# HongwenZhang/DaNet-DensePose2SMPL

Hardware: NVIDIA H100
Metric: images/sec DaNet fwd bs=64 224x224 (HRNet-W48 + part regressors + SMPL LBS + IUV render) (higher is better)
Workload: dtype split-f16 operands (hi+lo, 22 bits; 3 MMAs per K step), f32 accumulate

## Files before the change

### __graft_entry__.py

```python
import os
import subprocess
import sys

ROOT = os.path.dirname(os.path.abspath(__file__))
PKG = os.path.join(ROOT, "danet-densepose2smpl_b200")
CSRC = os.path.join(PKG, "csrc")
LIB = os.path.join(PKG, "libdanet_b200.so")
SOURCES = ["api.cu", "lbs.cu", "raster.cu", "glue.cu", "conv_simt.cu", "conv_tc.cu", "net.cu", "losses.cu", "iuv_train.cu",
           "gcn_train.cu", "conv_wgrad.cu", "bn_train.cu"]
ARCH = ["-gencode", "arch=compute_90a,code=sm_90a"]
NVCC_FLAGS = ARCH + [ "-lineinfo", "-O3", "-std=c++17",
              "-Xcompiler", "-fPIC", "--use_fast_math=false"]


def _stale(target, deps):
    if not os.path.exists(target):
        return True
    t = os.path.getmtime(target)
    return any(os.path.getmtime(d) > t for d in deps)


def build(verbose=False):
    nvcc = os.environ.get("NVCC", "/usr/local/cuda/bin/nvcc")
    hdrs = [os.path.join(CSRC, "common.cuh"), os.path.join(ROOT, "include", "danet_b200.h")]
# ... 9 lines not shown
            subprocess.check_call(cmd)
        objs.append(o)
    if _stale(LIB, objs):
        subprocess.check_call([nvcc, "-shared"] + ARCH + ["-o", LIB] + objs + ["-lcudart"])
    exe = os.path.join(ROOT, "examples", "net_host")
    if _stale(exe, [exe + ".c", LIB, os.path.join(ROOT, "include", "danet_b200.h")]):
        subprocess.check_call(["gcc", "-O2", "-I" + os.path.join(ROOT, "include"), exe + ".c", "-o", exe, "-L" + PKG, "-ldanet_b200",
                               "-Wl,-rpath,$ORIGIN/../" + os.path.basename(PKG)])
    subprocess.check_call(["make", "-s", "-C", os.path.join(ROOT, "oracle"), "liboracle.so"])
    if os.path.isdir("/root/reference/models/danet") and not os.path.exists(os.path.join(ROOT, "oracle", "_ref", ".complete")):
        subprocess.check_call([sys.executable, "-m", "oracle.make_ref"], cwd=ROOT)
    if ROOT not in sys.path:
        sys.path.insert(0, ROOT)
    import danet_b200
    return LIB


def smoke():
    if ROOT not in sys.path:
        sys.path.insert(0, ROOT)
    import numpy as np
    import torch
    import danet_b200
    from oracle import synth, lbs as olbs, raster as oraster

    assert torch.cuda.is_available(), "smoke() needs a GPU"
    dev = torch.device("cuda:0")
    model = synth.make_smpl_model(0)
    mesh = synth.make_dp_mesh(0)
    smpl = danet_b200.SMPL(model, batch_size=4).to(dev)
# ... 24 lines not shown
    assert plan.n_tc > 300 and plan.precision == "exact", "smoke must run the tensor-core path"
    kps_err = float((out["stn_kps_pred"].cpu() - torch.from_numpy(g["stn_kps"])).abs().max())
    idx = out["visualization"]["iuv_pred"][2].argmax(1).cpu().numpy()
    parts = out["visualization"]["part_iuv_pred"][:, :, 2].argmax(2).cpu().numpy()
    clean = ~((idx != g["index_argmax"]).reshape(2, -1).any(1) | (parts != g["part_argmax"]).reshape(2, -1).any(1))
    perr = np.abs(out["para"].cpu().numpy() - g["para"]).max(1)
    assert kps_err < 1e-4, kps_err
    assert clean.any() and perr[clean].max() < 1e-4, (perr, clean)
    torch.cuda.synchronize()
    print("smoke ok: verts max|d|=%.2e joints max|d|=%.2e, IUV parts bit-exact, network para max|d|=%.2e (wgmma exact mode, "
          "%d convolutions) vs the reference golden" % (dv, dj, perr[clean].max(), plan.n_tc))


if __name__ == "__main__":
    build(verbose="-v" in sys.argv)
    if "smoke" in sys.argv:
        smoke()
```

### danet-densepose2smpl_b200/csrc/conv_tc.cu

```cuda
#include "common.cuh"
#include "wgmma_f16.cuh"
#include "tc_ptx.cuh"
#include <cuda.h>
#include <cuda_fp16.h>
#include <mutex>
#include <type_traits>
#include <utility>
#include <string.h>
#include <math.h>

namespace danet {
namespace tc {

constexpr int kTileH = 16, kTileW = 8;
__host__ __device__ constexpr int kConsumersOf(int ex) { return ex ? 4 : 2; }
__host__ __device__ constexpr int kThreadsOf(int ex) { return ex ? 4 * 4 * 32 : (4 * 2 + 1) * 32; }
constexpr int kWarpProd = 4 * kConsumersOf(0);
constexpr int kNtMaxExact = 64, kNtMaxFast = 256;
constexpr int kMaxAStages = 8, kMaxBStages = 8;
constexpr int kSmemMax = 227 * 1024;
constexpr int kSmemFixed = 2048;
constexpr int kSchedDepth = 4, kSchedAhead = 2, kSchedStatic = 3;
__host__ __device__ constexpr int kSchedConsumersOf(int ex) { return 4 * kConsumersOf(ex); }
constexpr int kPackHeader = 1024;
constexpr int kSegMmas = 8;

struct alignas(64) Prob {
    CUtensorMap tm[2];
    const uint8_t* wpk; const float* bias;
    const float* res_f; const __half* res_hi; const __half* res_lo;
    float* y_f; __half* y_hi; __half* y_lo;
    int N, H, W, Cin, Cout, Ho, Wo, ks, stride, pad, relu, wsets, exact;
    int npa;
    int SWB, KCH, nchunks;
    int TG;
    int NT, ntn;
    int nstack, hs, box_h;
    int bpc;
    int par_py[4], par_px[4], ntap[4], ngrp[4], stage_bytes[4], sbo_a[4];
    int tapoff16[4][16];
    int tapidx[4][16];
    int tiles_w, tiles_h, tile_count, tile_base;
    int rows_blk;
    int tap_bytes, b_block_bytes, nblk;
    long long blocks_per_set;
    unsigned long long m_ntn, m_tw, m_th, m_ws;
};

constexpr int kMaxProb = 6;
struct ArgsN {
    int nprob, total_tiles, na_stages, a_slot_bytes, nb_stages, b_slot_bytes;
    unsigned* sched;
    Prob p[kMaxProb];
    int pair_base[kMaxProb], pair_count[kMaxProb], total_pairs;
};

static unsigned long long magic40(int d) { return (1ull << 40) / (unsigned long long)d + 1ull; }

static bool make_prob(const danet_conv_desc* d, Prob* g) {
    if (!(d->stride == 1 || d->stride == 2) || !(d->ksize == 1 || d->ksize == 3 || d->ksize == 7) || d->pad != d->ksize / 2) return false;
    if (d->Cin % 8 != 0 || d->Cout % 8 != 0 || d->H < 1 || d->W < 1 || d->N < 1 || d->wsets < 1) return false;
    g->N = d->N; g->H = d->H; g->W = d->W; g->Cin = d->Cin; g->Cout = d->Cout; g->ks = d->ksize;
    g->pad = d->pad; g->stride = d->stride; g->relu = d->relu; g->wsets = d->wsets;
    g->exact = (d->flags & DANET_CONV_EXACT) ? 1 : 0;
    g->Ho = (d->H + 2 * d->pad - d->ksize) / d->stride + 1;
    g->Wo = (d->W + 2 * d->pad - d->ksize) / d->stride + 1;
    if (g->Ho < 1 || g->Wo < 1) return false;
    const int np = (d->Cout + 15) / 16 * 16;
    const int ntmax = g->exact ? kNtMaxExact : kNtMaxFast;
// ... 71 lines not shown
}

static bool plan_rings(ArgsN* a) {
    int amax = 0, bmax = 0, need_a = 2, max_a = kMaxAStages;
    bool exact = false;
    for (int i = 0; i < a->nprob; ++i) {
        const int sb = max_stage_bytes(a->p[i]);
        amax = sb > amax ? sb : amax;
        bmax = a->p[i].b_block_bytes > bmax ? a->p[i].b_block_bytes : bmax;
        if (a->p[i].exact) exact = true;
    }
    a->a_slot_bytes = (amax + 1023) / 1024 * 1024;
    a->b_slot_bytes = (bmax + 1023) / 1024 * 1024;
    if (exact) {
        a->a_slot_bytes *= 2;
        need_a = max_a = 3;
    }
    int nb = 3;
    int na = (kSmemMax - kSmemFixed - nb * a->b_slot_bytes) / a->a_slot_bytes;
    if (na < need_a) { nb = 2; na = (kSmemMax - kSmemFixed - nb * a->b_slot_bytes) / a->a_slot_bytes; }
    if (na < need_a) return false;
    if (na > max_a) na = max_a;
    while (nb < kMaxBStages && kSmemFixed + na * a->a_slot_bytes + (nb + 1) * a->b_slot_bytes <= kSmemMax) ++nb;
    a->na_stages = na; a->nb_stages = nb;
    return true;
}

__device__ __forceinline__ uint64_t make_desc(uint32_t saddr, uint32_t sbo_bytes, uint32_t swb) {
    const uint32_t mode = swb == 128 ? 1u : (swb == 64 ? 2u : 3u);
    const uint32_t lo = ((saddr >> 4) & 0x3FFFu) | (1u << 16);
    const uint32_t hi = ((sbo_bytes >> 4) & 0x3FFFu) | (mode << 30);
// ... 31 lines not shown
    if (g.tiles_h > 1) {
        const int th2 = (g.tiles_h + 1) >> 1;
        grp = outer / th2;
        c.th = 2 * (outer - grp * th2) + h;
    } else {
        const int q = mdiv(outer, g.m_ws);
        grp = (2 * q + h) * g.wsets + (outer - q * g.wsets);
        c.th = 0;
    }
    const int bg = mdiv(grp, g.m_ws);
    c.ws = grp - bg * g.wsets;
    c.img0 = c.ws + g.wsets * bg * g.nstack;
    return c;
}

struct Ring { int as, bs; uint32_t aph, bph; };

struct Smem { uint32_t sA, sB, bar_a_full, bar_a_empty, bar_b_full, bar_b_empty; };

constexpr uint32_t kOffSchedFull = 512, kOffSchedEmpty = kOffSchedFull + 8 * kSchedDepth;
constexpr uint32_t kOffSchedRing = kOffSchedFull + 16 * kSchedDepth, kOffCursor = 640, kOffPark = 768;

enum CursorField {
    kCurSeq, kCurPub, kCurPubEnd,
    kCurPi,
    kCurC, kCurSlot, kCurStep,
    kCurH0, kCurH1, kCurW0,
    kCurImg0, kCurImg1, kCurBlk,
    kCurFa, kCurFb,
    kCurRa, kCurRb,
    kCurAs, kCurBs, kCurAph, kCurBph,
    kCurFields
};
static_assert(kOffCursor + 4 * kCurFields <= kOffPark && kOffPark + 4 * 32 <= 1024, "barrier region layout");
__device__ __forceinline__ int cur_get(uint32_t cur, int f) {
    int v;
    asm volatile("ld.shared.s32 %0, [%1];" : "=r"(v) : "r"(cur + 4 * f) : "memory");
    return v;
}
__device__ __forceinline__ void cur_set(uint32_t cur, int f, int v) {
    asm volatile("st.shared.s32 [%0], %1;" ::"r"(cur + 4 * f), "r"(v) : "memory");
}

__device__ __forceinline__ void produce(const ArgsN& a, const Smem& S, int dA, int dB) {
    const uint32_t cur = S.bar_a_full + kOffCursor;
    cur_set(cur, kCurRa, cur_get(cur, kCurRa) + dA);
    cur_set(cur, kCurRb, cur_get(cur, kCurRb) + dB);
#pragma unroll 1
    for (;;) {
        if (cur_get(cur, kCurPi) < 0) {
#pragma unroll 1
            while (cur_get(cur, kCurPub) <= cur_get(cur, kCurSeq) + kSchedAhead && !cur_get(cur, kCurPubEnd)) {
                const int pub = cur_get(cur, kCurPub), rs = pub & (kSchedDepth - 1);
                mbar_wait_inl(S.bar_a_full + kOffSchedEmpty + 8 * rs, ((pub / kSchedDepth) & 1) ^ 1);
                int t;
                if (pub < kSchedStatic || !a.sched) t = (int)blockIdx.x + pub * (int)gridDim.x;
                else t = __shfl_sync(0xffffffffu, atom_inc_elect(a.sched), 0) + kSchedStatic * (int)gridDim.x;
                if (t >= a.total_pairs) { t = a.total_pairs; cur_set(cur, kCurPubEnd, 1); }
                st_arrive_elect(S.bar_a_full + kOffSchedRing + 4 * rs, t, S.bar_a_full + kOffSchedFull + 8 * rs);
                cur_set(cur, kCurPub, pub + 1);
            }
            int pair;
            asm volatile("ld.shared.s32 %0, [%1];" : "=r"(pair)
                         : "r"(S.bar_a_full + kOffSchedRing + 4 * (cur_get(cur, kCurSeq) & (kSchedDepth - 1))) : "memory");
            pair = __shfl_sync(0xffffffffu, pair, 0);
            if (pair >= a.total_pairs) return;
            int pi = 0;
            while (pair >= a.pair_base[pi] + a.pair_count[pi]) ++pi;
            const Prob& P = a.p[pi];
            const int pp = pair - a.pair_base[pi];
            {
                const TileCoord tc = pair_coord(P, pp, 0);
                cur_set(cur, kCurH0, tc.th * kTileH * P.stride - P.pad);
                cur_set(cur, kCurW0, tc.tw * kTileW * P.stride - P.pad);
                cur_set(cur, kCurImg0, tc.img0);
                cur_set(cur, kCurBlk, tc.ws * (int)P.blocks_per_set + tc.nt * P.nblk);
            }
            {
                const TileCoord tc = pair_coord(P, pp, 1);
                cur_set(cur, kCurH1, tc.th * kTileH * P.stride - P.pad);
                cur_set(cur, kCurImg1, tc.img0);
            }
            cur_set(cur, kCurC, 0); cur_set(cur, kCurSlot, 0); cur_set(cur, kCurStep, 0);
            cur_set(cur, kCurPi, pi);
        }
        const Prob& P = a.p[cur_get(cur, kCurPi)];
        const int step = cur_get(cur, kCurStep);
        if (step < 2) {
            if (cur_get(cur, kCurFa) >= cur_get(cur, kCurRa) + a.na_stages) return;
            {
                const int as = cur_get(cur, kCurAs);
                mbar_wait_inl(S.bar_a_empty + 8 * as, ((cur_get(cur, kCurAph) >> as) & 1) ^ 1);
                mbar_expect_tx_elect(S.bar_a_full + 8 * as, 2u * P.nstack * P.box_h * P.sbo_a[cur_get(cur, kCurSlot)]);
            }
#pragma unroll 1
            for (int k = 0; k < 2 * P.nstack; ++k) {
                const int h = k >= P.nstack ? 1 : 0, n = k - h * P.nstack, slot = cur_get(cur, kCurSlot), as = cur_get(cur, kCurAs);
                tma_load_4d_elect(S.sA + as * a.a_slot_bytes + h * (a.a_slot_bytes >> 1) + n * P.hs * P.sbo_a[slot],
                                  &P.tm[step], cur_get(cur, kCurC) * P.KCH, cur_get(cur, kCurW0) + P.par_px[slot],
                                  cur_get(cur, kCurH0 + h) + P.par_py[slot], cur_get(cur, kCurImg0 + h) + n * P.wsets,
                                  S.bar_a_full + 8 * as);
            }
            const int as = cur_get(cur, kCurAs);
            cur_set(cur, kCurAph, cur_get(cur, kCurAph) ^ (1 << as));
            cur_set(cur, kCurAs, as + 1 == a.na_stages ? 0 : as + 1);
            cur_set(cur, kCurFa, cur_get(cur, kCurFa) + 1);
            cur_set(cur, kCurStep, step + 1);
        } else {
            if (cur_get(cur, kCurFb) >= cur_get(cur, kCurRb) + a.nb_stages) return;
            {
                const int bs = cur_get(cur, kCurBs);
                mbar_wait_inl(S.bar_b_empty + 8 * bs, ((cur_get(cur, kCurBph) >> bs) & 1) ^ 1);
                const uint32_t bar = S.bar_b_full + 8 * bs;
                mbar_expect_tx_elect(bar, (uint32_t)P.b_block_bytes);
                bulk_g2s_elect(S.sB + bs * a.b_slot_bytes, P.wpk + kPackHeader + (long long)cur_get(cur, kCurBlk) * P.b_block_bytes,
                               (uint32_t)P.b_block_bytes, bar);
                cur_set(cur, kCurBph, cur_get(cur, kCurBph) ^ (1 << bs));
                cur_set(cur, kCurBs, bs + 1 == a.nb_stages ? 0 : bs + 1);
            }
            cur_set(cur, kCurFb, cur_get(cur, kCurFb) + 1);
            cur_set(cur, kCurBlk, cur_get(cur, kCurBlk) + 1);
            const int slot = cur_get(cur, kCurSlot);
            if (step - 1 < P.ngrp[slot]) cur_set(cur, kCurStep, step + 1);
            else {
                cur_set(cur, kCurStep, 0);
                if (slot + 1 < P.npa) cur_set(cur, kCurSlot, slot + 1);
                else {
                    cur_set(cur, kCurSlot, 0);
                    if (cur_get(cur, kCurC) + 1 < P.nchunks) cur_set(cur, kCurC, cur_get(cur, kCurC) + 1);
                    else { cur_set(cur, kCurPi, -1); cur_set(cur, kCurSeq, cur_get(cur, kCurSeq) + 1); }
                }
            }
        }
    }
}

template <int EX, int NT>
__device__ __forceinline__ void consume_tile(const ArgsN& a, const Prob& P, const TileCoord tc, const Smem S, Ring& R,
                                             int wg, int w4, int lane, bool leader, float* accs, float* sum,
                                             int half = 0, bool prod = false) {
    constexpr int NV = NT / 2;
    constexpr int nj = NT / 8;
    const int prow0 = 8 * wg + 2 * w4, pcol = lane >> 2, cq = 2 * (lane & 3);
    float* s = accs;
    float* m = EX ? accs + NV : accs;
    const int Cout = P.Cout, Wo = P.Wo, Ho = P.Ho;
    const int cw = Cout - tc.nt * NT;
    uint32_t eoff[2]; bool ok[2];
    const int ow = tc.tw * kTileW + pcol;
#pragma unroll
    for (int r = 0; r < 2; ++r) {
        const int prow = prow0 + r;
        int oh = tc.th * kTileH + prow, img = tc.img0;
        bool row_ok = oh < Ho;
        if (P.nstack > 1) {
// ... 26 lines not shown
                    }
                }
            }
        }
        return t;
    };
    if constexpr (EX) {
#pragma unroll
        for (int j = 0; j < nj; ++j)
#pragma unroll
            for (int r = 0; r < 2; ++r) {
                const float2 t = init_term(j, r);
                sum[4 * j + 2 * r] = t.x * wsc.x; sum[4 * j + 2 * r + 1] = t.y * wsc.x;
            }
    }
    using Var = std::conditional_t<EX, int, const int>;
    Var nchunks = P.nchunks, npa = P.npa, TG = P.TG, SWB = P.SWB;
    Var kmma = P.KCH / 16;
    std::conditional_t<EX, int, const uint32_t> tap16 = P.tap_bytes >> 4;
    std::conditional_t<EX, int, const uint32_t> hi16 = EX ? (NT * SWB) >> 4 : 0;
    const uint64_t bd0 = make_desc(0, 8 * SWB, SWB);
    uint32_t acc = 0;
    int seg_cnt = 0;
    int pend_b = -1, pend_a = -1;
    auto release_pending = [&]() {
        mbar_arrive_if(S.bar_b_empty + 8 * pend_b, leader && pend_b >= 0);
        mbar_arrive_if(S.bar_a_empty + 8 * pend_a, leader && pend_a >= 0);
        pend_b = pend_a = -1;
    };
    for (int c = 0; c < nchunks; ++c) {
        const int kreal = (P.Cin - c * P.KCH + 15) >> 4;
        Var kv = kreal < kmma ? kreal : kmma;
        for (int slot = 0; slot < npa; ++slot) {
            Var as_hi = R.as;
            mbar_wait_inl(S.bar_a_full + 8 * R.as, (R.aph >> R.as) & 1u);
            R.aph ^= 1u << R.as; if (++R.as == a.na_stages) R.as = 0;
            int as_lo = as_hi;
            if (EX) {
                as_lo = R.as;
                mbar_wait_inl(S.bar_a_full + 8 * R.as, (R.aph >> R.as) & 1u);
                R.aph ^= 1u << R.as; if (++R.as == a.na_stages) R.as = 0;
            }
            const uint64_t ad0 = make_desc(0, (uint32_t)P.sbo_a[slot], SWB) + ((uint32_t)(wg * 8 * P.sbo_a[slot]) >> 4);
            const uint64_t ad_hi = ad0 + ((S.sA + as_hi * a.a_slot_bytes) >> 4);
            Var ngrp = P.ngrp[slot], ntap = P.ntap[slot];
            for (int tg = 0; tg < ngrp; ++tg) {
                const int k0 = tg * TG;
                const int ntk = min(TG, ntap - k0);
                const int bs = R.bs;
                mbar_wait_inl(S.bar_b_full + 8 * bs, (R.bph >> bs) & 1u);
                R.bph ^= 1u << bs; if (++R.bs == a.nb_stages) R.bs = 0;
                uint64_t bd;
                if constexpr (EX) bd = make_desc(0, 8 * SWB, SWB) + ((S.sB + bs * a.b_slot_bytes) >> 4);
                else bd = bd0 + ((S.sB + bs * a.b_slot_bytes) >> 4);
                wg_fence();
                if constexpr (EX) {
                    const uint32_t tile_a = S.sA + half * (a.a_slot_bytes >> 1) + wg * 8 * P.sbo_a[slot];
                    const uint64_t ad1 = make_desc(0, (uint32_t)P.sbo_a[slot], SWB);
                    const uint64_t ad_hi = ad1 + ((tile_a + as_hi * a.a_slot_bytes) >> 4);
                    const uint64_t ad_lo = ad1 + ((tile_a + as_lo * a.a_slot_bytes) >> 4);
                    #pragma unroll 1
                    for (int tt = 0; tt < ntk; ++tt) {
                        const uint32_t toff = (uint32_t)P.tapoff16[slot][k0 + tt];
                        #pragma unroll
                        for (int kk = 0; kk < 4; ++kk) {
// ... 12 lines not shown
                        }
                    }
                } else {
                    #pragma unroll 1
                    for (int tt = 0; tt < ntk; ++tt) {
                        const uint32_t toff = (uint32_t)P.tapoff16[slot][k0 + tt];
                        #pragma unroll
                        for (int kk = 0; kk < 4; ++kk) {
                            if (kk >= kv) break;
                            Wgmma<NT>::mma(m, m + NT / 4, ad_hi + toff + 2 * kk, bd + tt * tap16 + 2 * kk, acc);
                            acc = 1;
                        }
                    }
                }
                wg_commit();
                const bool plane_end = tg == ngrp - 1;
                if constexpr (EX) {
                    seg_cnt += ntk * kv;
                    const bool close = (c == nchunks - 1 && slot == npa - 1 && plane_end) || seg_cnt >= kSegMmas;
                    const int db = pend_b >= 0 ? 1 : 0;
                    int dA = 0, dB = db;
                    if (close || plane_end) {
                        wg_wait_all();
                        reg_fence<NV>(m);
                        reg_fence<NV>(s);
                        if (close) {
#pragma unroll
                            for (int j = 0; j < NV; ++j) {
                                sum[j] += m[j];
                                sum[j] += s[j];
                            }
                            acc = 0; seg_cnt = 0;
                        }
                        release_pending();
                        mbar_arrive_if(S.bar_b_empty + 8 * bs, leader);
                        mbar_arrive_if(S.bar_a_empty + 8 * as_hi, leader && plane_end);
                        mbar_arrive_if(S.bar_a_empty + 8 * as_lo, leader && plane_end);
                        dA = plane_end ? 2 : 0; dB = db + 1;
                    } else {
                        wg_wait_1();
                        release_pending();
                        pend_b = bs;
                    }
                    if (prod) {
                        const uint32_t pk = S.bar_a_full + kOffPark;
                        int* const v[] = {&c, &slot, &tg, &kv, &ngrp, &ntap, &as_hi, &as_lo, &seg_cnt, &pend_b, &R.as, &R.bs,
                                          &nchunks, &npa, &TG, &SWB, &kmma, &tap16, &hi16};
                        constexpr int nv = sizeof(v) / sizeof(v[0]);
#pragma unroll
                        for (int i = 0; i < nv; ++i) cur_set(pk, i, *v[i]);
                        cur_set(pk, nv, (int)acc); cur_set(pk, nv + 1, (int)R.aph); cur_set(pk, nv + 2, (int)R.bph);
                        produce(a, S, dA, dB);
#pragma unroll
                        for (int i = 0; i < nv; ++i) *v[i] = __shfl_sync(0xffffffffu, cur_get(pk, i), 0);
                        acc = (uint32_t)__shfl_sync(0xffffffffu, cur_get(pk, nv), 0);
                        R.aph = (uint32_t)__shfl_sync(0xffffffffu, cur_get(pk, nv + 1), 0);
                        R.bph = (uint32_t)__shfl_sync(0xffffffffu, cur_get(pk, nv + 2), 0);
                    }
                } else {
                    wg_wait_1();
                    release_pending();
                    pend_b = bs;
                    if (plane_end) pend_a = as_hi;
                }
            }
        }
    }
    wg_wait_all();
    reg_fence<NV>(m);
    if constexpr (EX) reg_fence<NV>(s);
    release_pending();
    const int relu = P.relu;
    float* __restrict__ y_f = P.y_f; __half* __restrict__ y_hi = P.y_hi; __half* __restrict__ y_lo = P.y_lo;
#pragma unroll
    for (int j = 0; j < nj; ++j) {
        if (8 * j >= cw) continue;
#pragma unroll
        for (int r = 0; r < 2; ++r) {
            if (!ok[r]) continue;
            float v0, v1;
            if constexpr (EX) { v0 = sum[4 * j + 2 * r]; v1 = sum[4 * j + 2 * r + 1]; }
            else {
                const float2 t = init_term(j, r);
                v0 = m[4 * j + 2 * r]; v1 = m[4 * j + 2 * r + 1];
                v0 += t.x * wsc.x; v1 += t.y * wsc.x;
            }
            float x0 = v0 * wsc.y, x1 = v1 * wsc.y;
            if (relu) { x0 = fmaxf(x0, 0.f); x1 = fmaxf(x1, 0.f); }
            const uint32_t e = eoff[r] + 8 * j;
            if (y_f) *reinterpret_cast<float2*>(y_f + e) = make_float2(x0, x1);
            if (y_hi) {
                const uint32_t hv = pack_h2_rn(x0, x1);
                *reinterpret_cast<uint32_t*>(y_hi + e) = hv;
                if (y_lo) {
                    const float2 t = h2_to_f2(hv);
                    *reinterpret_cast<uint32_t*>(y_lo + e) = pack_h2_rn(x0 - t.x, x1 - t.y);
                }
            }
        }
    }
}

template <int EX>
__global__ void __launch_bounds__(kThreadsOf(EX), 1)
k_conv_tc(const __grid_constant__ ArgsN a) {
    extern __shared__ __align__(1024) uint8_t smem[];
    const uint32_t sbase = (smem_u32(smem) + 1023u) & ~1023u;
    const uint32_t sA = sbase;
    const uint32_t sB = sbase + a.na_stages * a.a_slot_bytes;
    const uint32_t sBar = sB + a.nb_stages * a.b_slot_bytes;
    const uint32_t bar_a_full = sBar, bar_a_empty = sBar + 8 * kMaxAStages;
    const uint32_t bar_b_full = sBar + 16 * kMaxAStages, bar_b_empty = bar_b_full + 8 * kMaxBStages;
    const uint32_t bar_sched_full = sBar + kOffSchedFull, bar_sched_empty = sBar + kOffSchedEmpty, sched_ring = sBar + kOffSchedRing;
    constexpr int kCons = kConsumersOf(EX);

    const int warp = __shfl_sync(0xffffffffu, (int)(threadIdx.x >> 5), 0), lane = threadIdx.x & 31;
    if (threadIdx.x == 0) {
        for (int i = 0; i < a.na_stages; ++i) { mbar_init(bar_a_full + 8 * i, 1); mbar_init(bar_a_empty + 8 * i, kCons); }
        for (int i = 0; i < a.nb_stages; ++i) { mbar_init(bar_b_full + 8 * i, 1); mbar_init(bar_b_empty + 8 * i, kCons); }
        for (int i = 0; i < kSchedDepth; ++i) { mbar_init(bar_sched_full + 8 * i, 1); mbar_init(bar_sched_empty + 8 * i, kSchedConsumersOf(EX)); }
        asm volatile("fence.mbarrier_init.release.cluster;" ::: "memory");
        if constexpr (EX)
            for (int f = 0; f < kCurFields; ++f) cur_set(sBar + kOffCursor, f, f == kCurPi ? -1 : 0);
    }
    if (warp == (EX ? 0 : kWarpProd) && lane < a.nprob) { tma_prefetch_desc(&a.p[lane].tm[0]); if (EX) tma_prefetch_desc(&a.p[lane].tm[1]); }
    __syncthreads();
    pdl_launch_dependents();

    if constexpr (EX) {
        const int wg = warp >> 2, w4 = warp & 3;
        const bool leader = (threadIdx.x & 127) == 0;
        const bool prod = warp == 0;
        const Smem S = {sA, sB, bar_a_full, bar_a_empty, bar_b_full, bar_b_empty};
        Ring R = {0, 0, 0u, 0u};
        constexpr int NVMAX = kNtMaxExact / 2;
        float accs[2 * NVMAX];
        float sum[NVMAX];
        pdl_wait();
        if (prod) produce(a, S, 0, 0);
        for (int seq = 0;; ++seq) {
            int pair = 0;
            if (lane == 0) pair = sched_next(bar_sched_full, bar_sched_empty, sched_ring, seq);
            pair = __shfl_sync(0xffffffffu, pair, 0);
            if (pair >= a.total_pairs) break;
            int pi = 0;
            while (pair >= a.pair_base[pi] + a.pair_count[pi]) ++pi;
            const Prob& P = a.p[pi];
            const int half = wg >> 1;
            const TileCoord tc = pair_coord(P, pair - a.pair_base[pi], half);
#define DANET_NT_CASE(N) case N: consume_tile<EX, N>(a, P, tc, S, R, wg & 1, w4, lane, leader, accs, sum, half, prod); break;
            switch (P.NT) {
                DANET_NT_CASE(16) DANET_NT_CASE(32) DANET_NT_CASE(48) DANET_NT_CASE(64)
                default: __trap();
            }
#undef DANET_NT_CASE
        }
    } else if (warp == kWarpProd) {
        if (lane == 0) {
            int as = 0, bs = 0; uint32_t aph = 0, bph = 0;
            int pub = 0; bool ended = false;
            for (int seq = 0;; ++seq) {
                while (pub <= seq + kSchedAhead && !ended) {
                    const int slot = pub & (kSchedDepth - 1);
                    mbar_wait(bar_sched_empty + 8 * slot, ((pub / kSchedDepth) & 1) ^ 1);
                    int t;
                    if (pub < kSchedStatic || !a.sched) t = (int)blockIdx.x + pub * (int)gridDim.x;
                    else t = (int)atomicAdd(a.sched, 1u) + kSchedStatic * (int)gridDim.x;
                    if (t >= a.total_tiles) { t = a.total_tiles; ended = true; }
                    asm volatile("st.shared.s32 [%0], %1;" ::"r"(sched_ring + 4 * slot), "r"(t) : "memory");
                    mbar_arrive(bar_sched_full + 8 * slot);
// ... 35 lines not shown
                        }
                    }
            }
        }
    } else {
        const int wg = warp >> 2, w4 = warp & 3;
        const bool leader = (threadIdx.x & 127) == 0;
        const Smem S = {sA, sB, bar_a_full, bar_a_empty, bar_b_full, bar_b_empty};
        Ring R = {0, 0, 0u, 0u};
        float accs[kNtMaxFast / 2];
        pdl_wait();
        for (int seq = 0;; ++seq) {
            int tile = 0;
            if (lane == 0) tile = sched_next(bar_sched_full, bar_sched_empty, sched_ring, seq);
            tile = __shfl_sync(0xffffffffu, tile, 0);
            if (tile >= a.total_tiles) break;
            int pi = 0;
            while (tile >= a.p[pi].tile_base + a.p[pi].tile_count) ++pi;
            const Prob& P = a.p[pi];
            const TileCoord tc = decode_tile(P, tile - P.tile_base);
#define DANET_NT_CASE(N) case N: consume_tile<EX, N>(a, P, tc, S, R, wg, w4, lane, leader, accs, nullptr); break;
            switch (P.NT) {
                DANET_NT_CASE(16) DANET_NT_CASE(32) DANET_NT_CASE(48) DANET_NT_CASE(64) DANET_NT_CASE(80) DANET_NT_CASE(96)
                DANET_NT_CASE(112) DANET_NT_CASE(128) DANET_NT_CASE(144) DANET_NT_CASE(160) DANET_NT_CASE(176) DANET_NT_CASE(192)
                DANET_NT_CASE(208) DANET_NT_CASE(224) DANET_NT_CASE(240) DANET_NT_CASE(256)
                default: __trap();
            }
#undef DANET_NT_CASE
        }
    }
    __syncthreads();
    if (threadIdx.x == 0 && a.sched) {
        __threadfence();
        if (atomicAdd(a.sched + 1, 1u) == gridDim.x - 1) { a.sched[0] = 0u; a.sched[1] = 0u; __threadfence(); }
    }
}

__global__ void k_absmax(long long n, const float* __restrict__ w, unsigned* __restrict__ out) {
    unsigned m = 0;
    for (long long i = (long long)blockIdx.x * blockDim.x + threadIdx.x; i < n; i += (long long)gridDim.x * blockDim.x) {
        const unsigned b = __float_as_uint(fabsf(w[i]));
        if (b < 0x7f800000u && b > m) m = b;
    }
    for (int o = 16; o > 0; o >>= 1) m = max(m, __shfl_xor_sync(0xffffffffu, m, o));
    if ((threadIdx.x & 31) == 0 && m) atomicMax(out, m);
}
// ... 75 lines not shown
    const CUtensorMapSwizzle sw = g.SWB == 128 ? CU_TENSOR_MAP_SWIZZLE_128B : (g.SWB == 64 ? CU_TENSOR_MAP_SWIZZLE_64B : CU_TENSOR_MAP_SWIZZLE_32B);
    const CUresult r = fn(tm, CU_TENSOR_MAP_DATA_TYPE_FLOAT16, 4, const_cast<void*>(base), gdim, gstr, box, estr,
                          CU_TENSOR_MAP_INTERLEAVE_NONE, sw, CU_TENSOR_MAP_L2_PROMOTION_L2_128B, CU_TENSOR_MAP_FLOAT_OOB_FILL_NONE);
    DANET_CHECK(r == CUDA_SUCCESS, "conv_tc: cuTensorMapEncodeTiled failed (%d) for [%d,%d,%d,%d] box [%u,%u,%u]", (int)r,
                g.N, g.H, g.W, g.Cin, box[0], box[1], box[2]);
    return 0;
}

}

static int g_sm_count[64];
static unsigned* g_sched[64];
static unsigned g_sched_seq[64];
constexpr int kSchedSlots = 1024;
static std::mutex g_tc_mu;
static unsigned long long g_tc_devs = 0;

static int configure_group(int n, const danet_conv_desc* const* descs, tc::ArgsN* a) {
    using namespace tc;
    memset(a, 0, sizeof(*a));
    a->nprob = n;
    for (int i = 0; i < n; ++i)
        if (!make_prob(descs[i], &a->p[i])) { set_error("danet_conv_tc_group: problem %d has an unsupported shape", i); return -1; }
    for (int i = 1; i < n; ++i)
        DANET_CHECK(a->p[i].exact == a->p[0].exact, "danet_conv_tc_group: exact and fast problems cannot share a launch");
    DANET_CHECK(plan_rings(a), "danet_conv_tc_group: shared-memory plan does not fit");
    return 0;
}

int conv_tc_group_launch(int n, const danet_conv_problem* probs, cudaStream_t stream) {
// ... 40 lines not shown
    const int units = a.p[0].exact ? a.total_pairs : a.total_tiles;
    int dev = 0;
    DANET_CUDA(cudaGetDevice(&dev));
    DANET_CHECK(dev >= 0 && dev < 64, "conv_tc: device ordinal %d out of range", dev);
    {
        std::lock_guard<std::mutex> lk(g_tc_mu);
        if (first_use_on_current_device(&g_tc_devs) != 0) {
            DANET_CUDA(cudaDeviceGetAttribute(&g_sm_count[dev], cudaDevAttrMultiProcessorCount, dev));
            DANET_CUDA(cudaFuncSetAttribute(k_conv_tc<0>, cudaFuncAttributeMaxDynamicSharedMemorySize, kSmemMax));
            DANET_CUDA(cudaFuncSetAttribute(k_conv_tc<1>, cudaFuncAttributeMaxDynamicSharedMemorySize, kSmemMax));
            DANET_CUDA(cudaMalloc((void**)&g_sched[dev], kSchedSlots * 2 * sizeof(unsigned)));
            DANET_CUDA(cudaMemset(g_sched[dev], 0, kSchedSlots * 2 * sizeof(unsigned)));
        }
        a.sched = g_sched[dev] + 2 * (g_sched_seq[dev]++ % kSchedSlots);
    }
    const int smem_bytes = kSmemFixed + a.na_stages * a.a_slot_bytes + a.nb_stages * a.b_slot_bytes;
    const int cap = g_sm_count[dev];
    const int grid = units < cap ? units : cap;
    cudaLaunchConfig_t cfg = {};
    cfg.gridDim = dim3(grid); cfg.blockDim = dim3(kThreadsOf(a.p[0].exact));
    cfg.dynamicSmemBytes = smem_bytes;
    cfg.stream = stream;
    cudaLaunchAttribute at[1];
    at[0].id = cudaLaunchAttributeProgrammaticStreamSerialization;
    at[0].val.programmaticStreamSerializationAllowed = 1;
    cfg.attrs = at; cfg.numAttrs = 1;
    if (a.p[0].exact) { DANET_CUDA(cudaLaunchKernelEx(&cfg, k_conv_tc<1>, a)); }
    else { DANET_CUDA(cudaLaunchKernelEx(&cfg, k_conv_tc<0>, a)); }
    DANET_LAUNCH_CHECK();
    return 0;
// ... 90 lines not shown
extern "C" int danet_act_split(int64_t n, const float* x, void* hi, void* lo, danet_stream_t stream) {
    DANET_CHECK(n >= 0 && (n == 0 || (x && hi)), "danet_act_split: bad arguments");
    if (n == 0) return 0;
    tc::k_act_split<<<(unsigned)((n + 255) / 256), 256, 0, (cudaStream_t)stream>>>(n, x, (__half*)hi, (__half*)lo);
    DANET_LAUNCH_CHECK();
    return 0;
}

extern "C" int danet_act_merge(int64_t n, const void* hi, const void* lo, float* y, danet_stream_t stream) {
    DANET_CHECK(n >= 0 && (n == 0 || (hi && y)), "danet_act_merge: bad arguments");
    if (n == 0) return 0;
    tc::k_act_merge<<<(unsigned)((n + 255) / 256), 256, 0, (cudaStream_t)stream>>>(n, (const __half*)hi, (const __half*)lo, y);
    DANET_LAUNCH_CHECK();
    return 0;
}
```

Measured before the change: 1562.

## Pack producer cursor state, prefetch next schedule slot, add phase profiler build

Adds an optional phase-profiling build, off by default, that times each consumer phase with clock counters in shared memory. In the default path it also changes the exact-mode producer/consumer loop. Cursor fields are regrouped so they can be read and written with 128-bit shared loads and stores. The parked consumer state shrinks from about 22 words to two bit-packed words, with per-problem constants reloaded from the parameter struct. The next scheduler entry is now fetched before the epilogue rather than after it. The aim is to cut shared-memory traffic and scheduler latency in the interleaved producer role, at the risk of bit-field overflow if stage counts or chunk indices exceed the packed widths.

Result: faster. 1608 (median of 6 runs) (+2.9%).

```diff
diff --git a/__graft_entry__.py b/__graft_entry__.py
--- a/__graft_entry__.py
+++ b/__graft_entry__.py
@@ -47,6 +47,24 @@
         sys.path.insert(0, ROOT)
     import danet_b200
     return LIB
+
+
+PHASE_LIB = os.path.join(PKG, "libdanet_b200_phase.so")
+
+
+def build_phase_profile():
+    build()
+    nvcc = os.environ.get("NVCC", "/usr/local/cuda/bin/nvcc")
+    flags = [f for f in NVCC_FLAGS if not f.startswith("--use_fast_math")]
+    src = os.path.join(CSRC, "conv_tc.cu")
+    obj = os.path.join(PKG, "build", "conv_tc_phase.o")
+    hdrs = [os.path.join(ROOT, "include", "danet_b200.h")] + [os.path.join(CSRC, f) for f in os.listdir(CSRC) if f.endswith(".cuh")]
+    if _stale(obj, [src] + hdrs):
+        subprocess.check_call([nvcc] + flags + ["-DDANET_CONV_PHASE_PROFILE", "-c", src, "-o", obj])
+    objs = [obj if s == "conv_tc.cu" else os.path.join(PKG, "build", s.replace(".cu", ".o")) for s in SOURCES]
+    if _stale(PHASE_LIB, objs):
+        subprocess.check_call([nvcc, "-shared"] + ARCH + ["-o", PHASE_LIB] + objs + ["-lcudart"])
+    return PHASE_LIB
 
 
 def smoke():
@@ -101,5 +119,7 @@
 
 if __name__ == "__main__":
     build(verbose="-v" in sys.argv)
+    if "phase" in sys.argv:
+        build_phase_profile()
     if "smoke" in sys.argv:
         smoke()
diff --git a/danet-densepose2smpl_b200/csrc/conv_tc.cu b/danet-densepose2smpl_b200/csrc/conv_tc.cu
--- a/danet-densepose2smpl_b200/csrc/conv_tc.cu
+++ b/danet-densepose2smpl_b200/csrc/conv_tc.cu
@@ -19,10 +19,15 @@
 constexpr int kNtMaxExact = 64, kNtMaxFast = 256;
 constexpr int kMaxAStages = 8, kMaxBStages = 8;
 constexpr int kSmemMax = 227 * 1024;
+#ifdef DANET_CONV_PHASE_PROFILE
+constexpr int kSmemFixed = 4096;
+#else
 constexpr int kSmemFixed = 2048;
+#endif
 constexpr int kSchedDepth = 4, kSchedAhead = 2, kSchedStatic = 3;
 __host__ __device__ constexpr int kSchedConsumersOf(int ex) { return 4 * kConsumersOf(ex); }
 constexpr int kPackHeader = 1024;
+constexpr int kExactAStages = 3;
 constexpr int kSegMmas = 8;
 
 struct alignas(64) Prob {
@@ -53,6 +58,9 @@
     unsigned* sched;
     Prob p[kMaxProb];
     int pair_base[kMaxProb], pair_count[kMaxProb], total_pairs;
+#ifdef DANET_CONV_PHASE_PROFILE
+    unsigned long long* prof;
+#endif
 };
 
 static unsigned long long magic40(int d) { return (1ull << 40) / (unsigned long long)d + 1ull; }
@@ -154,7 +162,7 @@
     a->b_slot_bytes = (bmax + 1023) / 1024 * 1024;
     if (exact) {
         a->a_slot_bytes *= 2;
-        need_a = max_a = 3;
+        need_a = max_a = kExactAStages;
     }
     int nb = 3;
     int na = (kSmemMax - kSmemFixed - nb * a->b_slot_bytes) / a->a_slot_bytes;
@@ -216,6 +224,50 @@
     return c;
 }
 
+#define DANET_CONV_PHASES(X) \
+    X(Last) X(Start) X(Resident) X(Other) X(Sched) X(Prologue) X(WaitAHi) X(WaitALo) X(WaitB) X(Mma) X(Wait1) X(DrainSeg) X(DrainPlane) X(Sum) \
+    X(Park) X(Produce) X(ProduceSpin) X(Reload) X(Epilogue) X(Tail) X(Units) X(Blocks)
+enum Phase {
+#define X(n) kPh##n,
+    DANET_CONV_PHASES(X)
+#undef X
+    kPhN
+};
+#ifdef DANET_CONV_PHASE_PROFILE
+static_assert(kPhLast == 0 && kPhStart == 1 && kPhResident == 2 && kPhN <= 32, "one lane per phase");
+constexpr uint32_t kOffProf = 1024;
+static_assert(kOffProf + 16 * 4 * kPhN + 1023 <= kSmemFixed, "phase rows");
+__device__ __forceinline__ uint32_t prof_row(uint32_t sbar) { return sbar + kOffProf + (threadIdx.x >> 5) * (4 * kPhN); }
+__device__ __forceinline__ void prof_tick(uint32_t sbar, int ph) {
+    asm volatile("{\n\t.reg .u32 now, prev, sum;\n\tmov.u32 now, %%clock;\n\tld.shared.u32 prev, [%0];\n\tld.shared.u32 sum, [%1];\n\t"
+                 "sub.u32 prev, now, prev;\n\tadd.u32 sum, sum, prev;\n\tst.shared.u32 [%1], sum;\n\tst.shared.u32 [%0], now;\n\t}"
+                 ::"r"(prof_row(sbar)), "r"(prof_row(sbar) + 4 * ph) : "memory");
+}
+__device__ __forceinline__ void prof_count(uint32_t sbar, int ph) {
+    asm volatile("{\n\t.reg .u32 n;\n\tld.shared.u32 n, [%0];\n\tadd.u32 n, n, 1;\n\tst.shared.u32 [%0], n;\n\t}"
+                 ::"r"(prof_row(sbar) + 4 * ph) : "memory");
+}
+__device__ __forceinline__ void prof_start(uint32_t sbar) {
+    asm volatile("{\n\t.reg .pred p;\n\t.reg .u32 now;\n\tsetp.lt.u32 p, %1, %2;\n\t@p st.shared.u32 [%0], 0;\n\tbar.warp.sync 0xffffffff;\n\t"
+                 "mov.u32 now, %%clock;\n\tst.shared.u32 [%3], now;\n\tst.shared.u32 [%3 + 4], now;\n\t}"
+                 ::"r"(prof_row(sbar) + 4 * (threadIdx.x & 31)), "r"(threadIdx.x & 31), "r"((uint32_t)kPhN), "r"(prof_row(sbar)) : "memory");
+}
+__device__ __forceinline__ void prof_flush(uint32_t sbar, unsigned long long* tab, int pi) {
+    const uint32_t lane = threadIdx.x & 31;
+    unsigned long long* dst = tab + ((size_t)pi * 16 + (threadIdx.x >> 5)) * kPhN + lane;
+    const uint32_t on = lane > kPhStart && lane < kPhN && tab != nullptr;
+    asm volatile("{\n\t.reg .pred p;\n\t.reg .u32 v;\n\t.reg .u64 w;\n\tbar.warp.sync 0xffffffff;\n\tsetp.ne.u32 p, %1, 0;\n\t"
+                 "mov.u32 v, 0;\n\t@p ld.shared.u32 v, [%0];\n\tcvt.u64.u32 w, v;\n\t@p red.global.add.u64 [%2], w;\n\t"
+                 "@p st.shared.u32 [%0], 0;\n\tbar.warp.sync 0xffffffff;\n\t}"
+                 ::"r"(prof_row(sbar) + 4 * lane), "r"(on), "l"(dst) : "memory");
+}
+#define PROF_TICK(sbar, ph) prof_tick(sbar, ph)
+#define PROF_COUNT(sbar, ph) prof_count(sbar, ph)
+#else
+#define PROF_TICK(sbar, ph) ((void)0)
+#define PROF_COUNT(sbar, ph) ((void)0)
+#endif
+
 struct Ring { int as, bs; uint32_t aph, bph; };
 
 struct Smem { uint32_t sA, sB, bar_a_full, bar_a_empty, bar_b_full, bar_b_empty; };
@@ -224,17 +276,17 @@
 constexpr uint32_t kOffSchedRing = kOffSchedFull + 16 * kSchedDepth, kOffCursor = 640, kOffPark = 768;
 
 enum CursorField {
+    kCurPi, kCurStep, kCurSlot, kCurC,
+    kCurFb, kCurRb, kCurBs, kCurBph,
+    kCurFa, kCurRa, kCurAs, kCurAph,
+    kCurBlk, kCurW0, kCurH0, kCurH1,
+    kCurImg0, kCurImg1,
     kCurSeq, kCurPub, kCurPubEnd,
-    kCurPi,
-    kCurC, kCurSlot, kCurStep,
-    kCurH0, kCurH1, kCurW0,
-    kCurImg0, kCurImg1, kCurBlk,
-    kCurFa, kCurFb,
-    kCurRa, kCurRb,
-    kCurAs, kCurBs, kCurAph, kCurBph,
     kCurFields
 };
-static_assert(kOffCursor + 4 * kCurFields <= kOffPark && kOffPark + 4 * 32 <= 1024, "barrier region layout");
+static_assert(kOffCursor % 16 == 0 && kCurStep == kCurPi + 1 && kCurSlot == kCurPi + 2 && kCurC == kCurPi + 3 && kCurPi % 4 == 0 &&
+              kCurFb % 4 == 0 && kCurFa % 4 == 0, "cursor groups");
+static_assert(kOffCursor + 4 * kCurFields <= kOffPark && kOffPark + 4 * 2 <= 1024, "barrier region layout");
 __device__ __forceinline__ int cur_get(uint32_t cur, int f) {
     int v;
     asm volatile("ld.shared.s32 %0, [%1];" : "=r"(v) : "r"(cur + 4 * f) : "memory");
@@ -243,18 +295,29 @@
 __device__ __forceinline__ void cur_set(uint32_t cur, int f, int v) {
     asm volatile("st.shared.s32 [%0], %1;" ::"r"(cur + 4 * f), "r"(v) : "memory");
 }
+__device__ __forceinline__ int4 cur_get4(uint32_t cur, int f) {
+    int4 v;
+    asm volatile("ld.shared.v4.s32 {%0, %1, %2, %3}, [%4];" : "=r"(v.x), "=r"(v.y), "=r"(v.z), "=r"(v.w) : "r"(cur + 4 * f) : "memory");
+    return v;
+}
+__device__ __forceinline__ void cur_set4(uint32_t cur, int f, int4 v) {
+    asm volatile("st.shared.v4.s32 [%0], {%1, %2, %3, %4};" ::"r"(cur + 4 * f), "r"(v.x), "r"(v.y), "r"(v.z), "r"(v.w) : "memory");
+}
 
 __device__ __forceinline__ void produce(const ArgsN& a, const Smem& S, int dA, int dB) {
     const uint32_t cur = S.bar_a_full + kOffCursor;
-    cur_set(cur, kCurRa, cur_get(cur, kCurRa) + dA);
-    cur_set(cur, kCurRb, cur_get(cur, kCurRb) + dB);
+    if (dA) cur_set(cur, kCurRa, cur_get(cur, kCurRa) + dA);
+    if (dB) cur_set(cur, kCurRb, cur_get(cur, kCurRb) + dB);
 #pragma unroll 1
     for (;;) {
-        if (cur_get(cur, kCurPi) < 0) {
+        int4 ctl = cur_get4(cur, kCurPi);
+        if (ctl.x < 0) {
 #pragma unroll 1
             while (cur_get(cur, kCurPub) <= cur_get(cur, kCurSeq) + kSchedAhead && !cur_get(cur, kCurPubEnd)) {
                 const int pub = cur_get(cur, kCurPub), rs = pub & (kSchedDepth - 1);
+                PROF_TICK(S.bar_a_full, kPhProduce);
                 mbar_wait_inl(S.bar_a_full + kOffSchedEmpty + 8 * rs, ((pub / kSchedDepth) & 1) ^ 1);
+                PROF_TICK(S.bar_a_full, kPhProduceSpin);
                 int t;
                 if (pub < kSchedStatic || !a.sched) t = (int)blockIdx.x + pub * (int)gridDim.x;
                 else t = __shfl_sync(0xffffffffu, atom_inc_elect(a.sched), 0) + kSchedStatic * (int)gridDim.x;
@@ -283,56 +346,57 @@
                 cur_set(cur, kCurH1, tc.th * kTileH * P.stride - P.pad);
                 cur_set(cur, kCurImg1, tc.img0);
             }
-            cur_set(cur, kCurC, 0); cur_set(cur, kCurSlot, 0); cur_set(cur, kCurStep, 0);
-            cur_set(cur, kCurPi, pi);
-        }
-        const Prob& P = a.p[cur_get(cur, kCurPi)];
-        const int step = cur_get(cur, kCurStep);
-        if (step < 2) {
-            if (cur_get(cur, kCurFa) >= cur_get(cur, kCurRa) + a.na_stages) return;
-            {
-                const int as = cur_get(cur, kCurAs);
-                mbar_wait_inl(S.bar_a_empty + 8 * as, ((cur_get(cur, kCurAph) >> as) & 1) ^ 1);
-                mbar_expect_tx_elect(S.bar_a_full + 8 * as, 2u * P.nstack * P.box_h * P.sbo_a[cur_get(cur, kCurSlot)]);
-            }
+            ctl = make_int4(pi, 0, 0, 0);
+            cur_set4(cur, kCurPi, ctl);
+        }
+        const Prob& P = a.p[ctl.x];
+        if (ctl.y < 2) {
+            int4 ra = cur_get4(cur, kCurFa);
+            if (ra.x >= ra.y + a.na_stages) return;
+            PROF_TICK(S.bar_a_full, kPhProduce);
+            mbar_wait_inl(S.bar_a_empty + 8 * ra.z, ((ra.w >> ra.z) & 1) ^ 1);
+            PROF_TICK(S.bar_a_full, kPhProduceSpin);
+            mbar_expect_tx_elect(S.bar_a_full + 8 * ra.z, 2u * P.nstack * P.box_h * P.sbo_a[ctl.z]);
 #pragma unroll 1
             for (int k = 0; k < 2 * P.nstack; ++k) {
-                const int h = k >= P.nstack ? 1 : 0, n = k - h * P.nstack, slot = cur_get(cur, kCurSlot), as = cur_get(cur, kCurAs);
-                tma_load_4d_elect(S.sA + as * a.a_slot_bytes + h * (a.a_slot_bytes >> 1) + n * P.hs * P.sbo_a[slot],
-                                  &P.tm[step], cur_get(cur, kCurC) * P.KCH, cur_get(cur, kCurW0) + P.par_px[slot],
-                                  cur_get(cur, kCurH0 + h) + P.par_py[slot], cur_get(cur, kCurImg0 + h) + n * P.wsets,
-                                  S.bar_a_full + 8 * as);
-            }
-            const int as = cur_get(cur, kCurAs);
-            cur_set(cur, kCurAph, cur_get(cur, kCurAph) ^ (1 << as));
-            cur_set(cur, kCurAs, as + 1 == a.na_stages ? 0 : as + 1);
-            cur_set(cur, kCurFa, cur_get(cur, kCurFa) + 1);
-            cur_set(cur, kCurStep, step + 1);
+                const int h = k >= P.nstack ? 1 : 0, n = k - h * P.nstack;
+                tma_load_4d_elect(S.sA + ra.z * a.a_slot_bytes + h * (a.a_slot_bytes >> 1) + n * P.hs * P.sbo_a[ctl.z],
+                                  &P.tm[ctl.y], ctl.w * P.KCH, cur_get(cur, kCurW0) + P.par_px[ctl.z],
+                                  cur_get(cur, kCurH0 + h) + P.par_py[ctl.z], cur_get(cur, kCurImg0 + h) + n * P.wsets,
+                                  S.bar_a_full + 8 * ra.z);
+            }
+            ra.w ^= 1 << ra.z;
+            ra.z = ra.z + 1 == a.na_stages ? 0 : ra.z + 1;
+            ++ra.x;
+            cur_set4(cur, kCurFa, ra);
+            cur_set(cur, kCurStep, ctl.y + 1);
         } else {
-            if (cur_get(cur, kCurFb) >= cur_get(cur, kCurRb) + a.nb_stages) return;
-            {
-                const int bs = cur_get(cur, kCurBs);
-                mbar_wait_inl(S.bar_b_empty + 8 * bs, ((cur_get(cur, kCurBph) >> bs) & 1) ^ 1);
-                const uint32_t bar = S.bar_b_full + 8 * bs;
-                mbar_expect_tx_elect(bar, (uint32_t)P.b_block_bytes);
-                bulk_g2s_elect(S.sB + bs * a.b_slot_bytes, P.wpk + kPackHeader + (long long)cur_get(cur, kCurBlk) * P.b_block_bytes,
-                               (uint32_t)P.b_block_bytes, bar);
-                cur_set(cur, kCurBph, cur_get(cur, kCurBph) ^ (1 << bs));
-                cur_set(cur, kCurBs, bs + 1 == a.nb_stages ? 0 : bs + 1);
-            }
-            cur_set(cur, kCurFb, cur_get(cur, kCurFb) + 1);
-            cur_set(cur, kCurBlk, cur_get(cur, kCurBlk) + 1);
-            const int slot = cur_get(cur, kCurSlot);
-            if (step - 1 < P.ngrp[slot]) cur_set(cur, kCurStep, step + 1);
+            int4 rb = cur_get4(cur, kCurFb);
+            if (rb.x >= rb.y + a.nb_stages) return;
+            const int blk = cur_get(cur, kCurBlk);
+            PROF_TICK(S.bar_a_full, kPhProduce);
+            mbar_wait_inl(S.bar_b_empty + 8 * rb.z, ((rb.w >> rb.z) & 1) ^ 1);
+            PROF_TICK(S.bar_a_full, kPhProduceSpin);
+            const uint32_t bar = S.bar_b_full + 8 * rb.z;
+            mbar_expect_tx_elect(bar, (uint32_t)P.b_block_bytes);
+            bulk_g2s_elect(S.sB + rb.z * a.b_slot_bytes, P.wpk + kPackHeader + (long long)blk * P.b_block_bytes,
+                           (uint32_t)P.b_block_bytes, bar);
+            cur_set(cur, kCurBlk, blk + 1);
+            rb.w ^= 1 << rb.z;
+            rb.z = rb.z + 1 == a.nb_stages ? 0 : rb.z + 1;
+            ++rb.x;
+            cur_set4(cur, kCurFb, rb);
+            if (ctl.y - 1 < P.ngrp[ctl.z]) ++ctl.y;
             else {
-                cur_set(cur, kCurStep, 0);
-                if (slot + 1 < P.npa) cur_set(cur, kCurSlot, slot + 1);
+                ctl.y = 0;
+                if (ctl.z + 1 < P.npa) ++ctl.z;
                 else {
-                    cur_set(cur, kCurSlot, 0);
-                    if (cur_get(cur, kCurC) + 1 < P.nchunks) cur_set(cur, kCurC, cur_get(cur, kCurC) + 1);
-                    else { cur_set(cur, kCurPi, -1); cur_set(cur, kCurSeq, cur_get(cur, kCurSeq) + 1); }
+                    ctl.z = 0;
+                    if (ctl.w + 1 < P.nchunks) ++ctl.w;
+                    else { ctl.x = -1; ctl.w = 0; cur_set(cur, kCurSeq, cur_get(cur, kCurSeq) + 1); }
                 }
             }
+            cur_set4(cur, kCurPi, ctl);
         }
     }
 }
@@ -340,7 +404,7 @@
 template <int EX, int NT>
 __device__ __forceinline__ void consume_tile(const ArgsN& a, const Prob& P, const TileCoord tc, const Smem S, Ring& R,
                                              int wg, int w4, int lane, bool leader, float* accs, float* sum,
-                                             int half = 0, bool prod = false) {
+                                             int half = 0, bool prod = false, int seq = 0, int* next = nullptr) {
     constexpr int NV = NT / 2;
     constexpr int nj = NT / 8;
     const int prow0 = 8 * wg + 2 * w4, pcol = lane >> 2, cq = 2 * (lane & 3);
@@ -397,6 +461,7 @@
                 sum[4 * j + 2 * r] = t.x * wsc.x; sum[4 * j + 2 * r + 1] = t.y * wsc.x;
             }
     }
+    PROF_TICK(S.bar_a_full, kPhPrologue);
     using Var = std::conditional_t<EX, int, const int>;
     Var nchunks = P.nchunks, npa = P.npa, TG = P.TG, SWB = P.SWB;
     Var kmma = P.KCH / 16;
@@ -415,13 +480,15 @@
         const int kreal = (P.Cin - c * P.KCH + 15) >> 4;
         Var kv = kreal < kmma ? kreal : kmma;
         for (int slot = 0; slot < npa; ++slot) {
-            Var as_hi = R.as;
+            int as_hi = R.as;
             mbar_wait_inl(S.bar_a_full + 8 * R.as, (R.aph >> R.as) & 1u);
+            PROF_TICK(S.bar_a_full, kPhWaitAHi);
             R.aph ^= 1u << R.as; if (++R.as == a.na_stages) R.as = 0;
             int as_lo = as_hi;
             if (EX) {
                 as_lo = R.as;
                 mbar_wait_inl(S.bar_a_full + 8 * R.as, (R.aph >> R.as) & 1u);
+                PROF_TICK(S.bar_a_full, kPhWaitALo);
                 R.aph ^= 1u << R.as; if (++R.as == a.na_stages) R.as = 0;
             }
             const uint64_t ad0 = make_desc(0, (uint32_t)P.sbo_a[slot], SWB) + ((uint32_t)(wg * 8 * P.sbo_a[slot]) >> 4);
@@ -432,6 +499,8 @@
                 const int ntk = min(TG, ntap - k0);
                 const int bs = R.bs;
                 mbar_wait_inl(S.bar_b_full + 8 * bs, (R.bph >> bs) & 1u);
+                PROF_TICK(S.bar_a_full, kPhWaitB);
+                PROF_COUNT(S.bar_a_full, kPhBlocks);
                 R.bph ^= 1u << bs; if (++R.bs == a.nb_stages) R.bs = 0;
                 uint64_t bd;
                 if constexpr (EX) bd = make_desc(0, 8 * SWB, SWB) + ((S.sB + bs * a.b_slot_bytes) >> 4);
@@ -474,6 +543,7 @@
                     }
                 }
                 wg_commit();
+                PROF_TICK(S.bar_a_full, kPhMma);
                 const bool plane_end = tg == ngrp - 1;
                 if constexpr (EX) {
                     seg_cnt += ntk * kv;
@@ -482,6 +552,7 @@
                     int dA = 0, dB = db;
                     if (close || plane_end) {
                         wg_wait_all();
+                        PROF_TICK(S.bar_a_full, close ? kPhDrainSeg : kPhDrainPlane);
                         reg_fence<NV>(m);
                         reg_fence<NV>(s);
                         if (close) {
@@ -497,31 +568,42 @@
                         mbar_arrive_if(S.bar_a_empty + 8 * as_hi, leader && plane_end);
                         mbar_arrive_if(S.bar_a_empty + 8 * as_lo, leader && plane_end);
                         dA = plane_end ? 2 : 0; dB = db + 1;
+                        PROF_TICK(S.bar_a_full, kPhSum);
                     } else {
                         wg_wait_1();
                         release_pending();
                         pend_b = bs;
+                        PROF_TICK(S.bar_a_full, kPhWait1);
                     }
                     if (prod) {
+                        static_assert(kMaxBStages <= 8 && kMaxProb <= 8 && kSegMmas <= 16 && kExactAStages <= 4,
+                                      "bit fields of the parked words");
                         const uint32_t pk = S.bar_a_full + kOffPark;
-                        int* const v[] = {&c, &slot, &tg, &kv, &ngrp, &ntap, &as_hi, &as_lo, &seg_cnt, &pend_b, &R.as, &R.bs,
-                                          &nchunks, &npa, &TG, &SWB, &kmma, &tap16, &hi16};
-                        constexpr int nv = sizeof(v) / sizeof(v[0]);
-#pragma unroll
-                        for (int i = 0; i < nv; ++i) cur_set(pk, i, *v[i]);
-                        cur_set(pk, nv, (int)acc); cur_set(pk, nv + 1, (int)R.aph); cur_set(pk, nv + 2, (int)R.bph);
+                        cur_set(pk, 0, slot | tg << 2 | as_hi << 6 | as_lo << 8 | R.as << 10 | R.bs << 12 | c << 15);
+                        cur_set(pk, 1, (int)(R.aph | R.bph << 8 | (uint32_t)seg_cnt << 16 | (uint32_t)(pend_b + 1) << 20 | acc << 24 |
+                                           (uint32_t)(&P - a.p) << 25));
+                        PROF_TICK(S.bar_a_full, kPhPark);
                         produce(a, S, dA, dB);
-#pragma unroll
-                        for (int i = 0; i < nv; ++i) *v[i] = __shfl_sync(0xffffffffu, cur_get(pk, i), 0);
-                        acc = (uint32_t)__shfl_sync(0xffffffffu, cur_get(pk, nv), 0);
-                        R.aph = (uint32_t)__shfl_sync(0xffffffffu, cur_get(pk, nv + 1), 0);
-                        R.bph = (uint32_t)__shfl_sync(0xffffffffu, cur_get(pk, nv + 2), 0);
+                        PROF_TICK(S.bar_a_full, kPhProduce);
+                        const uint32_t w0 = (uint32_t)__shfl_sync(0xffffffffu, cur_get(pk, 0), 0);
+                        const uint32_t w1 = (uint32_t)__shfl_sync(0xffffffffu, cur_get(pk, 1), 0);
+                        slot = w0 & 3; tg = (w0 >> 2) & 15; as_hi = (w0 >> 6) & 3; as_lo = (w0 >> 8) & 3;
+                        R.as = (w0 >> 10) & 3; R.bs = (w0 >> 12) & 7; c = (int)(w0 >> 15);
+                        R.aph = w1 & 255u; R.bph = (w1 >> 8) & 255u; seg_cnt = (w1 >> 16) & 15;
+                        pend_b = (int)((w1 >> 20) & 15) - 1; acc = (w1 >> 24) & 1u;
+                        const Prob& Q = a.p[(w1 >> 25) & 7];
+                        nchunks = Q.nchunks; npa = Q.npa; TG = Q.TG; SWB = Q.SWB; kmma = Q.KCH / 16;
+                        tap16 = Q.tap_bytes >> 4; hi16 = (NT * SWB) >> 4;
+                        ngrp = Q.ngrp[slot]; ntap = Q.ntap[slot];
+                        kv = min((Q.Cin - c * Q.KCH + 15) >> 4, kmma);
+                        PROF_TICK(S.bar_a_full, kPhReload);
                     }
                 } else {
                     wg_wait_1();
                     release_pending();
                     pend_b = bs;
                     if (plane_end) pend_a = as_hi;
+                    PROF_TICK(S.bar_a_full, kPhWait1);
                 }
             }
         }
@@ -530,6 +612,13 @@
     reg_fence<NV>(m);
     if constexpr (EX) reg_fence<NV>(s);
     release_pending();
+    PROF_TICK(S.bar_a_full, EX ? kPhOther : kPhDrainPlane);
+    if constexpr (EX) {
+        int nx = 0;
+        if (lane == 0) nx = sched_next(S.bar_a_full + kOffSchedFull, S.bar_a_full + kOffSchedEmpty, S.bar_a_full + kOffSchedRing, seq + 1);
+        *next = __shfl_sync(0xffffffffu, nx, 0);
+        PROF_TICK(S.bar_a_full, kPhSched);
+    }
     const int relu = P.relu;
     float* __restrict__ y_f = P.y_f; __half* __restrict__ y_hi = P.y_hi; __half* __restrict__ y_lo = P.y_lo;
 #pragma unroll
@@ -559,6 +648,8 @@
             }
         }
     }
+    PROF_TICK(S.bar_a_full, kPhEpilogue);
+    PROF_COUNT(S.bar_a_full, kPhUnits);
 }
 
 template <int EX>
@@ -585,6 +676,9 @@
     }
     if (warp == (EX ? 0 : kWarpProd) && lane < a.nprob) { tma_prefetch_desc(&a.p[lane].tm[0]); if (EX) tma_prefetch_desc(&a.p[lane].tm[1]); }
     __syncthreads();
+#ifdef DANET_CONV_PHASE_PROFILE
+    prof_start(sBar);
+#endif
     pdl_launch_dependents();
 
     if constexpr (EX) {
@@ -597,23 +691,30 @@
         float accs[2 * NVMAX];
         float sum[NVMAX];
         pdl_wait();
+        PROF_TICK(sBar, kPhOther);
         if (prod) produce(a, S, 0, 0);
-        for (int seq = 0;; ++seq) {
-            int pair = 0;
-            if (lane == 0) pair = sched_next(bar_sched_full, bar_sched_empty, sched_ring, seq);
-            pair = __shfl_sync(0xffffffffu, pair, 0);
-            if (pair >= a.total_pairs) break;
+        PROF_TICK(sBar, kPhProduce);
+        int pair = 0;
+        if (lane == 0) pair = sched_next(bar_sched_full, bar_sched_empty, sched_ring, 0);
+        pair = __shfl_sync(0xffffffffu, pair, 0);
+        PROF_TICK(sBar, kPhSched);
+        for (int seq = 0; pair < a.total_pairs; ++seq) {
+            int next = 0;
             int pi = 0;
             while (pair >= a.pair_base[pi] + a.pair_count[pi]) ++pi;
             const Prob& P = a.p[pi];
             const int half = wg >> 1;
             const TileCoord tc = pair_coord(P, pair - a.pair_base[pi], half);
-#define DANET_NT_CASE(N) case N: consume_tile<EX, N>(a, P, tc, S, R, wg & 1, w4, lane, leader, accs, sum, half, prod); break;
+#define DANET_NT_CASE(N) case N: consume_tile<EX, N>(a, P, tc, S, R, wg & 1, w4, lane, leader, accs, sum, half, prod, seq, &next); break;
             switch (P.NT) {
                 DANET_NT_CASE(16) DANET_NT_CASE(32) DANET_NT_CASE(48) DANET_NT_CASE(64)
                 default: __trap();
             }
 #undef DANET_NT_CASE
+#ifdef DANET_CONV_PHASE_PROFILE
+            prof_flush(sBar, a.prof, pi);
+#endif
+            pair = next;
         }
     } else if (warp == kWarpProd) {
         if (lane == 0) {
@@ -679,6 +780,7 @@
             int tile = 0;
             if (lane == 0) tile = sched_next(bar_sched_full, bar_sched_empty, sched_ring, seq);
             tile = __shfl_sync(0xffffffffu, tile, 0);
+            PROF_TICK(sBar, kPhSched);
             if (tile >= a.total_tiles) break;
             int pi = 0;
             while (tile >= a.p[pi].tile_base + a.p[pi].tile_count) ++pi;
@@ -692,9 +794,18 @@
                 default: __trap();
             }
 #undef DANET_NT_CASE
+#ifdef DANET_CONV_PHASE_PROFILE
+            prof_flush(sBar, a.prof, pi);
+#endif
         }
     }
     __syncthreads();
+#ifdef DANET_CONV_PHASE_PROFILE
+    PROF_TICK(sBar, kPhTail);
+    asm volatile("{\n\t.reg .u32 t0, t1;\n\tld.shared.u32 t0, [%0];\n\tld.shared.u32 t1, [%0 + 4];\n\tsub.u32 t0, t0, t1;\n\t"
+                 "st.shared.u32 [%0 + 8], t0;\n\t}" ::"r"(prof_row(sBar)) : "memory");
+    prof_flush(sBar, a.prof, kMaxProb);
+#endif
     if (threadIdx.x == 0 && a.sched) {
         __threadfence();
         if (atomicAdd(a.sched + 1, 1u) == gridDim.x - 1) { a.sched[0] = 0u; a.sched[1] = 0u; __threadfence(); }
@@ -800,6 +911,9 @@
 static unsigned g_sched_seq[64];
 constexpr int kSchedSlots = 1024;
 static std::mutex g_tc_mu;
+#ifdef DANET_CONV_PHASE_PROFILE
+static unsigned long long* g_phase_table;
+#endif
 static unsigned long long g_tc_devs = 0;
 
 static int configure_group(int n, const danet_conv_desc* const* descs, tc::ArgsN* a) {
@@ -870,6 +984,9 @@
         }
         a.sched = g_sched[dev] + 2 * (g_sched_seq[dev]++ % kSchedSlots);
     }
+#ifdef DANET_CONV_PHASE_PROFILE
+    a.prof = g_phase_table;
+#endif
     const int smem_bytes = kSmemFixed + a.na_stages * a.a_slot_bytes + a.nb_stages * a.b_slot_bytes;
     const int cap = g_sm_count[dev];
     const int grid = units < cap ? units : cap;
@@ -990,3 +1107,13 @@
     DANET_LAUNCH_CHECK();
     return 0;
 }
+
+#ifdef DANET_CONV_PHASE_PROFILE
+extern "C" int danet_conv_phase_table(unsigned long long* table) { g_phase_table = table; return 0; }
+extern "C" const char* danet_conv_phase_layout(int32_t* dims) {
+    if (dims) { dims[0] = tc::kMaxProb + 1; dims[1] = 16; dims[2] = tc::kPhN; }
+#define X(n) #n ","
+    return DANET_CONV_PHASES(X);
+#undef X
+}
+#endif
```
